# SobeyMIL/MVOC

Measured on AMD Instinct MI355X. Metric: UNet3D denoising steps/sec, 16x512^2 frames, inversion+compose, higher is better.
Workload: dtype f16

## Files before the change

mvoc_amd/csrc/attention.hip:

```cpp
#include <stdlib.h>

#include "common.h"

namespace {

typedef __fp16 fp16x4_t __attribute__((__vector_size__(4 * sizeof(__fp16))));
template <int D> struct FlashPitch { static constexpr int K = 2 * D + 16, V = D == 64 ? 192 : 320; };

struct AttnArgs {
  const half_t *q, *k, *v;
  half_t* out;
  long q_bs, q_ts, k_bs, k_ts, v_bs, v_ts, o_bs, o_ts;
  int nbatch, heads, tq, tk, kv_bdiv, causal;
  float scale_log2;
  long v2_off, o2_off;
  int qblocks;
};

__device__ __forceinline__ int vt_slot_group(int key) {
  return ((((key >> 5) * 2 + ((key >> 4) & 1)) * 2) + ((key >> 2) & 1));
}
__device__ __forceinline__ int vt_slot_elem(int key) { return ((key >> 3) & 1) * 4 + (key & 3); }

constexpr float FLASH_THR = 8.0f;

typedef float f32x2 __attribute__((ext_vector_type(2)));
__device__ __forceinline__ float flash_xhalf_max(float x) {
  const unsigned u = __builtin_bit_cast(unsigned, x);
  const auto sw = __builtin_amdgcn_permlane32_swap(u, u, false, false);
  return fmaxf(__builtin_bit_cast(float, (unsigned)sw[0]), __builtin_bit_cast(float, (unsigned)sw[1]));
}

template <int D, int NV>
#ifndef FLASH_MINW
#define FLASH_MINW 4
#endif
__global__ __launch_bounds__(256, (D == 64 && NV == 1) ? FLASH_MINW : 1) void flash_kernel(const AttnArgs p) {
  constexpr int KPITCH = FlashPitch<D>::K, VPITCH = FlashPitch<D>::V;
  constexpr int ND = D / 16, NT = D / 32, CPK = D / 8, NCH = 64 * CPK / 256;
  __shared__ __attribute__((aligned(16))) char smem[64 * KPITCH + NV * 64 * VPITCH];
  char* Ks = smem;
  char* Vs = smem + 64 * KPITCH;
  const int tid = threadIdx.x, lane = tid & 63;
  const int wave = __builtin_amdgcn_readfirstlane(tid >> 6);
  const int r = lane & 31, h = lane >> 5;
  const unsigned logical = xcd_remap(blockIdx.x, gridDim.x);
  const unsigned qb_ = logical % (unsigned)p.qblocks, hb_ = logical / (unsigned)p.qblocks;
  const int head = (int)(hb_ % (unsigned)p.heads), b = (int)(hb_ / (unsigned)p.heads);
  const int q0 = (int)qb_ * 128 + wave * 32;

  const half_t* qp = p.q + (long)b * p.q_bs + head * D;
  const int qrow = min(q0 + r, p.tq - 1);
  half8_t qf[ND];
#pragma unroll
  for (int s = 0; s < ND; ++s) qf[s] = *reinterpret_cast<const half8_t*>(qp + (long)qrow * p.q_ts + 16 * s + 8 * h);

  const char* kb = reinterpret_cast<const char*>(p.k + (long)(b / p.kv_bdiv) * p.k_bs + head * D);
  const char* vb = reinterpret_cast<const char*>(p.v + (long)(b / p.kv_bdiv) * p.v_bs + head * D);
  const unsigned k_rb = (unsigned)p.k_ts * 2u, v_rb = (unsigned)p.v_ts * 2u;
  unsigned koff[NCH], voff[NCH];
#pragma unroll
  for (int i = 0; i < NCH; ++i) {
    const int c = tid + i * 256;
    koff[i] = (unsigned)(c / CPK) * k_rb + (unsigned)(c % CPK) * 16u;
    voff[i] = (unsigned)(c / CPK) * v_rb + (unsigned)(c % CPK) * 16u;
  }

  f32x16 ot[NV][NT];
#pragma unroll
  for (int v = 0; v < NV; ++v)
#pragma unroll
    for (int dt = 0; dt < NT; ++dt)
#pragma unroll
      for (int e = 0; e < 16; ++e) ot[v][dt][e] = 0.f;
  float mrun = -INFINITY, lrun = 0.f;

  const int ntiles = (p.tk + 63) / 64;
  half8_t kreg[NCH], vreg[NV][NCH];
  auto gload = [&](int kt) {
    const char* kt_ = kb + (size_t)kt * 64u * k_rb;
    const char* vt_ = vb + (size_t)kt * 64u * v_rb;
    const bool ragged = __builtin_amdgcn_readfirstlane(kt * 64 + 64 > p.tk);
#pragma unroll
    for (int i = 0; i < NCH; ++i) {
      unsigned ko = koff[i], vo = voff[i];
      if (ragged) {
        const int c = tid + i * 256;
        const unsigned row = (unsigned)min(c / CPK, p.tk - 1 - kt * 64);
        ko = row * k_rb + (unsigned)(c % CPK) * 16u;
        vo = row * v_rb + (unsigned)(c % CPK) * 16u;
      }
      kreg[i] = *reinterpret_cast<const half8_t*>(kt_ + ko);
#pragma unroll
      for (int v = 0; v < NV; ++v) vreg[v][i] = *reinterpret_cast<const half8_t*>(vt_ + (size_t)v * (size_t)p.v2_off * 2u + vo);
    }
  };
  gload(0);
  for (int kt = 0; kt < ntiles; ++kt) {
    __syncthreads();
#pragma unroll
    for (int i = 0; i < NCH; ++i) {
      const int c = tid + i * 256;
      const int key = c / CPK, dc = c % CPK;
      *reinterpret_cast<half8_t*>(Ks + key * KPITCH + dc * 16) = kreg[i];
#pragma unroll
      for (int v = 0; v < NV; ++v)
        *reinterpret_cast<half8_t*>(Vs + v * 64 * VPITCH + key * VPITCH + dc * 16) = vreg[v][i];
    }
    __syncthreads();
    if (kt + 1 < ntiles) gload(kt + 1);

    f32x16 st[2];
#pragma unroll
    for (int t = 0; t < 2; ++t) {
#pragma unroll
      for (int e = 0; e < 16; ++e) st[t][e] = 0.f;
#pragma unroll
      for (int s = 0; s < ND; ++s) {
        const half8_t kf = *reinterpret_cast<const half8_t*>(Ks + (32 * t + r) * KPITCH + (16 * s + 8 * h) * 2);
        st[t] = __builtin_amdgcn_mfma_f32_32x32x16_f16(kf, qf[s], st[t], 0, 0, 0);
      }
    }
    if (__builtin_amdgcn_readfirstlane((kt == ntiles - 1) && (p.tk & 63))) {
#pragma unroll
      for (int t = 0; t < 2; ++t)
#pragma unroll
        for (int e = 0; e < 16; ++e)
          if (kt * 64 + 32 * t + 8 * (e >> 2) + 4 * h + (e & 3) >= p.tk) st[t][e] = -INFINITY;
    }
    if (p.causal) {
#pragma unroll
      for (int t = 0; t < 2; ++t)
#pragma unroll
        for (int e = 0; e < 16; ++e)
          if (kt * 64 + 32 * t + 8 * (e >> 2) + 4 * h + (e & 3) > q0 + r) st[t][e] = -INFINITY;
    }
    float mx = st[0][0];
#pragma unroll
    for (int t = 0; t < 2; ++t)
#pragma unroll
      for (int e = 0; e < 16; ++e) mx = fmaxf(mx, st[t][e]);
    mx = flash_xhalf_max(mx);
    if (__any((mx - mrun) * p.scale_log2 > FLASH_THR)) {
      const float mnew = fmaxf(mrun, mx);
      const float alpha = __builtin_amdgcn_exp2f((mrun - mnew) * p.scale_log2);
      mrun = mnew;
      lrun *= alpha;
#pragma unroll
      for (int v = 0; v < NV; ++v)
#pragma unroll
        for (int dt = 0; dt < NT; ++dt)
#pragma unroll
          for (int e = 0; e < 16; ++e) ot[v][dt][e] *= alpha;
    }
    const f32x2 sc2 = {p.scale_log2, p.scale_log2}, mc2 = {-mrun * p.scale_log2, -mrun * p.scale_log2};
#pragma unroll
    for (int t = 0; t < 2; ++t)
#pragma unroll
      for (int e = 0; e < 16; e += 2) {
        const f32x2 a = __builtin_elementwise_fma(f32x2{st[t][e], st[t][e + 1]}, sc2, mc2);
        st[t][e] = __builtin_amdgcn_exp2f(a[0]);
        st[t][e + 1] = __builtin_amdgcn_exp2f(a[1]);
      }

#pragma unroll
    for (int t = 0; t < 2; ++t)
#pragma unroll
      for (int s = 0; s < 2; ++s) {
        half8_t pf;
#pragma unroll
        for (int j = 0; j < 8; ++j) pf[j] = (half_t)st[t][8 * s + j];
#pragma unroll
        for (int j = 0; j < 4; ++j) lrun = __builtin_amdgcn_fdot2(half2_t{pf[2 * j], pf[2 * j + 1]}, half2_t{(half_t)1.f, (half_t)1.f}, lrun, false);
        const int krow = 32 * t + 16 * s + 4 * h + ((lane & 15) >> 2);
#pragma unroll
        for (int v = 0; v < NV; ++v)
#pragma unroll
          for (int dt = 0; dt < NT; ++dt) {
            const char* va = Vs + v * 64 * VPITCH + krow * VPITCH + (32 * dt + 16 * ((lane >> 4) & 1) + 4 * (lane & 3)) * 2;
            const fp16x4_t lo = __builtin_amdgcn_ds_read_tr16_b64_v4f16((__attribute__((address_space(3))) fp16x4_t*)va);
            const fp16x4_t hi = __builtin_amdgcn_ds_read_tr16_b64_v4f16((__attribute__((address_space(3))) fp16x4_t*)(va + 8 * VPITCH));
            half8_t vf;
#pragma unroll
            for (int e = 0; e < 4; ++e) {
              vf[e] = (half_t)lo[e];
              vf[4 + e] = (half_t)hi[e];
            }
            ot[v][dt] = __builtin_amdgcn_mfma_f32_32x32x16_f16(vf, pf, ot[v][dt], 0, 0, 0);
          }
      }
  }
  const float ltot = lrun + __shfl_xor(lrun, 32);
  const float inv = 1.0f / ltot;
  int lane_e = tid;
  asm volatile("" : "+v"(lane_e));
  const int r_e = lane_e & 31, h_e = (lane_e >> 5) & 1;
  if (q0 + r_e < p.tq) {
#pragma unroll
    for (int v = 0; v < NV; ++v) {
      half_t* op = p.out + v * p.o2_off + (long)b * p.o_bs + (long)(q0 + r_e) * p.o_ts + head * D;
#pragma unroll
      for (int dt = 0; dt < NT; ++dt)
#pragma unroll
        for (int q = 0; q < 4; ++q) {
          half4_t o;
#pragma unroll
          for (int e = 0; e < 4; ++e) o[e] = (half_t)(ot[v][dt][q * 4 + e] * inv);
          *reinterpret_cast<half4_t*>(op + 32 * dt + 8 * q + 4 * h_e) = o;
        }
    }
  }
}

#define F3_BAR()                         \
  do {                                   \
    __builtin_amdgcn_sched_barrier(0);   \
    __builtin_amdgcn_s_barrier();        \
    __builtin_amdgcn_sched_barrier(0);   \
  } while (0)
#define F3_FENCE() __builtin_amdgcn_sched_barrier(0)
#define F3_GRP(V, T)                                   \
  do {                                                 \
    __builtin_amdgcn_sched_group_barrier(0x008, 1, 0); \
    __builtin_amdgcn_sched_group_barrier(0x002, V, 0); \
    __builtin_amdgcn_sched_group_barrier(0x400, T, 0); \
  } while (0)
#define F3_RD(R) __builtin_amdgcn_sched_group_barrier(0x100, R, 0)
#ifdef MVOC_F3_STAMPS
__device__ unsigned long long f3_dbg[8];
#define F3_STAMP(i)                                                                      \
  do {                                                                                   \
    unsigned long long t_;                                                               \
    asm volatile("s_memtime %0\n\ts_waitcnt lgkmcnt(0)" : "=s"(t_)::"memory");          \
    if (blockIdx.x == 0 && tid == 0) { f3_acc[i] += t_ - f3_last; }                      \
    f3_last = t_;                                                                        \
  } while (0)
#else
#define F3_STAMP(i)
#endif
typedef unsigned u32x4 __attribute__((ext_vector_type(4)));
__device__ __forceinline__ void f3_dma(const u32x4 rsrc, unsigned voff, unsigned lds) {
  unsigned keep;
  asm volatile("s_mov_b32 %0, m0\n\ts_mov_b32 m0, %2\n\ts_nop 0\n\tbuffer_load_dwordx4 %1, %3, 0 offen lds\n\ts_mov_b32 m0, %0"
               : "=&s"(keep) : "v"(voff), "s"(lds), "s"(rsrc) : "memory");
}
__device__ __forceinline__ u32x4 f3_rsrc(const void* base, unsigned bytes) {
  const unsigned long long a = (unsigned long long)base;
  u32x4 r;
  r[0] = __builtin_amdgcn_readfirstlane((unsigned)a);
  r[1] = __builtin_amdgcn_readfirstlane((unsigned)(a >> 32));
  r[2] = __builtin_amdgcn_readfirstlane(bytes);
  r[3] = 0x00020000u;
  return r;
}
template <int N>
__device__ __forceinline__ void f3_wait_vm() {
  asm volatile("s_waitcnt vmcnt(%0)" ::"n"(N) : "memory");
}
#ifndef F3_W1
#define F3_W1 3
#endif
template <int NV>
__global__ __launch_bounds__(256, NV == 1 ? F3_W1 : 2) void flash3_kernel(const AttnArgs p) {
  constexpr int D = 64, NS = (NV == 1 && F3_W1 == 2) ? 4 : 3, TILE = 8192 * (1 + NV), PCS = 2 + 2 * NV;
  __shared__ __attribute__((aligned(1024))) char smem[NS * TILE];
#ifdef MVOC_F3_STAMPS
  unsigned long long f3_acc[6] = {0, 0, 0, 0, 0, 0}, f3_last = 0, f3_t0, f3_r0;
#endif
  const int tid = threadIdx.x, lane = tid & 63;
  const int wave = __builtin_amdgcn_readfirstlane(tid >> 6);
  const int r = lane & 31, h = lane >> 5;
#ifdef MVOC_F3_STAMPS
  asm volatile("s_memtime %0\n\ts_memrealtime %1\n\ts_waitcnt lgkmcnt(0)" : "=s"(f3_t0), "=s"(f3_r0)::"memory");
  f3_last = f3_t0;
#endif
  const unsigned logical = xcd_remap(blockIdx.x, gridDim.x);
  const unsigned qb_ = logical % (unsigned)p.qblocks, hb_ = logical / (unsigned)p.qblocks;
  const int head = (int)(hb_ % (unsigned)p.heads), b = (int)(hb_ / (unsigned)p.heads);
  const int q0 = (int)qb_ * 128 + wave * 32;
  const int nt = (p.tk + 63) >> 6;

  const unsigned k_rb = (unsigned)p.k_ts * 2u, v_rb = (unsigned)p.v_ts * 2u;
  const half_t* kb = p.k + (long)(b / p.kv_bdiv) * p.k_bs + head * D;
  const half_t* vb = p.v + (long)(b / p.kv_bdiv) * p.v_bs + head * D;
  const u32x4 rs_k = f3_rsrc(kb, (unsigned)(p.tk - 1) * k_rb + 128u);
  const u32x4 rs_v0 = f3_rsrc(vb, (unsigned)(p.tk - 1) * v_rb + 128u);
  const u32x4 rs_v1 = f3_rsrc(vb + p.v2_off, (unsigned)(p.tk - 1) * v_rb + 128u);
  unsigned ksrc[2], vsrc[2];
#pragma unroll
  for (int j = 0; j < 2; ++j) {
    const int key_l = 16 * wave + 8 * j + (lane >> 3), pc = lane & 7;
    ksrc[j] = (unsigned)key_l * k_rb + (unsigned)((pc ^ ((key_l >> 1) & 7)) * 16);
    vsrc[j] = (unsigned)key_l * v_rb + (unsigned)((pc ^ (((key_l >> 1) & 1) << 2)) * 16);
  }
  const unsigned ktile = 64u * k_rb, vtile = 64u * v_rb;
  const unsigned lds0 = (unsigned)(size_t)(__attribute__((address_space(3))) char*)smem;
  auto issue = [&](int tile, int so) {
    const unsigned base = lds0 + (unsigned)so + (unsigned)wave * 2048u;
#pragma unroll
    for (int j = 0; j < 2; ++j) f3_dma(rs_k, ksrc[j] + (unsigned)tile * ktile, base + j * 1024);
#pragma unroll
    for (int v = 0; v < NV; ++v)
#pragma unroll
      for (int j = 0; j < 2; ++j) f3_dma(v ? rs_v1 : rs_v0, vsrc[j] + (unsigned)tile * vtile, base + 8192 * (1 + v) + j * 1024);
  };
  const half_t* qp = p.q + (long)b * p.q_bs + head * D;
  const int qrow = min(q0 + r, p.tq - 1);
  half8_t qf[4];
#pragma unroll
  for (int s = 0; s < 4; ++s) qf[s] = *reinterpret_cast<const half8_t*>(qp + (long)qrow * p.q_ts + 16 * s + 8 * h);
  asm volatile("s_nop 4" ::: "memory");
  F3_FENCE();
#pragma unroll
  for (int t = 0; t < NS - 1; ++t) issue(t, t * TILE);
  F3_FENCE();

  f32x16 ot[NV][2];
#pragma unroll
  for (int v = 0; v < NV; ++v)
#pragma unroll
    for (int dt = 0; dt < 2; ++dt)
#pragma unroll
      for (int e = 0; e < 16; ++e) ot[v][dt][e] = 0.f;
  float mrun = -INFINITY, lrun = 0.f;
  f32x16 sa[2], sb[2];
  f32x16 zero16;
#pragma unroll
  for (int e = 0; e < 16; ++e) zero16[e] = 0.f;

  int kfo[4];
#pragma unroll
  for (int s = 0; s < 4; ++s) kfo[s] = r * 128 + (((2 * s + h) ^ ((r >> 1) & 7)) * 16);
  const int vq = (lane & 15) >> 2;
  int vfo[2];
#pragma unroll
  for (int dt = 0; dt < 2; ++dt) vfo[dt] = 8192 + (4 * h + vq) * 128 + (((32 * ((lane >> 4) & 1) + 8 * (lane & 3))) | ((dt ^ ((vq >> 1) & 1)) << 6));

  f3_wait_vm<(NS - 2) * PCS>();
  F3_BAR();
#pragma unroll
  for (int t = 0; t < 2; ++t) {
    sa[t] = zero16;
#pragma unroll
    for (int s = 0; s < 4; ++s) {
      const half8_t kf = *reinterpret_cast<const half8_t*>(smem + kfo[s] + 4096 * t);
      sa[t] = __builtin_amdgcn_mfma_f32_32x32x16_f16(kf, qf[s], sa[t], 0, 0, 0);
    }
  }
  int o_v = 0, o_k = TILE, o_w = (NS - 1) * TILE;

  auto body = [&](f32x16(&cur)[2], f32x16(&nxt)[2], const int t) {
    F3_STAMP(4);
    f3_wait_vm<(NS - 3) * PCS>();
    F3_BAR();
    F3_STAMP(0);
    issue(t + NS - 1, o_w);
    F3_FENCE();
    F3_STAMP(1);
    const char* Kn = smem + o_k;
    const char* Vc = smem + o_v;
    if (__builtin_amdgcn_readfirstlane((t == nt - 1) && (p.tk & 63))) {
#pragma unroll
      for (int tt = 0; tt < 2; ++tt)
#pragma unroll
        for (int e = 0; e < 16; ++e)
          if (t * 64 + 32 * tt + 8 * (e >> 2) + 4 * h + (e & 3) >= p.tk) cur[tt][e] = -INFINITY;
    }
    F3_FENCE();
    half8_t kf[2][4];
#pragma unroll
    for (int s = 0; s < 2; ++s)
#pragma unroll
      for (int tt = 0; tt < 2; ++tt) kf[tt][s] = *reinterpret_cast<const half8_t*>(Kn + kfo[s] + 4096 * tt);
    half8_t pf[2];
    half8_t vf[3][NV][2];
    auto vread = [&](const int f) {
#pragma unroll
      for (int v = 0; v < NV; ++v)
#pragma unroll
        for (int dt = 0; dt < 2; ++dt) {
          const char* va = Vc + 8192 * v + vfo[dt] + (32 * (f >> 1) + 16 * (f & 1)) * 128;
          const fp16x4_t lo = __builtin_amdgcn_ds_read_tr16_b64_v4f16((__attribute__((address_space(3))) fp16x4_t*)va);
          const fp16x4_t hi = __builtin_amdgcn_ds_read_tr16_b64_v4f16((__attribute__((address_space(3))) fp16x4_t*)(va + 8 * 128));
#pragma unroll
          for (int e = 0; e < 4; ++e) {
            vf[f % 3][v][dt][e] = (half_t)lo[e];
            vf[f % 3][v][dt][4 + e] = (half_t)hi[e];
          }
        }
    };
    vread(0);
    F3_FENCE();
    auto smma = [&](const int i) {
      const int tt = i & 1, s_ = i >> 1;
      nxt[tt] = __builtin_amdgcn_mfma_f32_32x32x16_f16(kf[tt][s_], qf[s_], s_ == 0 ? zero16 : nxt[tt], 0, 0, 0);
    };
    auto pvmma = [&](const int f, const int dt) {
#pragma unroll
      for (int v = 0; v < NV; ++v) ot[v][dt] = __builtin_amdgcn_mfma_f32_32x32x16_f16(vf[f % 3][v][dt], pf[f & 1], ot[v][dt], 0, 0, 0);
    };
    float mx = fmaxf(cur[0][0], cur[0][1]);
#pragma unroll
    for (int tt = 0; tt < 2; ++tt)
#pragma unroll
      for (int e = tt ? 0 : 2; e < 16; e += 2) mx = __builtin_fmaxf(__builtin_fmaxf(mx, cur[tt][e]), cur[tt][e + 1]);
    smma(0); smma(1); smma(2);
    if constexpr (NV == 2) smma(3);
    mx = flash_xhalf_max(mx);
    if constexpr (NV == 1) { F3_GRP(6, 0); F3_GRP(6, 0); F3_GRP(6, 0); }
    else { F3_GRP(4, 0); F3_GRP(5, 0); F3_GRP(4, 0); F3_GRP(5, 0); }
    F3_STAMP(2);
    if (__any((mx - mrun) * p.scale_log2 > FLASH_THR)) {
      const float mnew = fmaxf(mrun, mx);
      const float alpha = __builtin_amdgcn_exp2f((mrun - mnew) * p.scale_log2);
      mrun = mnew;
      lrun *= alpha;
#pragma unroll
      for (int v = 0; v < NV; ++v)
#pragma unroll
        for (int dt = 0; dt < 2; ++dt)
#pragma unroll
          for (int e = 0; e < 16; ++e) ot[v][dt][e] *= alpha;
    }
    F3_FENCE();
    const f32x2 sc2 = {p.scale_log2, p.scale_log2}, mc2 = {-mrun * p.scale_log2, -mrun * p.scale_log2};
#pragma unroll
    for (int s = 2; s < 4; ++s)
#pragma unroll
      for (int tt = 0; tt < 2; ++tt) kf[tt][s] = *reinterpret_cast<const half8_t*>(Kn + kfo[s] + 4096 * tt);
#pragma unroll
    for (int f = 0; f < 4; ++f) {
      const int tt = f >> 1, s_ = f & 1;
      if (f < 3) vread(f + 1);
      half8_t& pn = pf[f & 1];
      float x[8];
#pragma unroll
      for (int j = 0; j < 8; j += 2) {
        const f32x2 a = __builtin_elementwise_fma(f32x2{cur[tt][8 * s_ + j], cur[tt][8 * s_ + j + 1]}, sc2, mc2);
        x[j] = __builtin_amdgcn_exp2f(a[0]);
        x[j + 1] = __builtin_amdgcn_exp2f(a[1]);
      }
#pragma unroll
      for (int j = 0; j < 8; ++j) pn[j] = (half_t)x[j];
#pragma unroll
      for (int j = 0; j < 4; ++j) lrun = __builtin_amdgcn_fdot2(half2_t{pn[2 * j], pn[2 * j + 1]}, half2_t{(half_t)1.f, (half_t)1.f}, lrun, false);
      if (f == 0) {
        smma(NV == 1 ? 3 : 4); smma(NV == 1 ? 4 : 5);
        if constexpr (NV == 2) { smma(6); smma(7); } else smma(5);
      } else {
        pvmma(f - 1, 0); pvmma(f - 1, 1);
        if constexpr (NV == 1) { if (f < 3) smma(5 + f); }
      }
    }
    pvmma(3, 0);
    pvmma(3, 1);
    if constexpr (NV == 1) {
      F3_RD(8); F3_GRP(5, 3); F3_GRP(5, 2); F3_GRP(5, 3);
      F3_RD(4); F3_GRP(5, 2); F3_GRP(5, 3); F3_GRP(5, 2);
      F3_RD(4); F3_GRP(5, 3); F3_GRP(5, 2); F3_GRP(5, 3);
      F3_GRP(5, 2); F3_GRP(5, 3); F3_GRP(5, 2); F3_GRP(5, 2);
    } else {
      F3_RD(12); F3_GRP(3, 2); F3_GRP(3, 2); F3_GRP(3, 2); F3_GRP(3, 2);
      F3_RD(8); F3_GRP(3, 2); F3_GRP(3, 2); F3_GRP(3, 2); F3_GRP(3, 2);
      F3_RD(8); F3_GRP(3, 2); F3_GRP(3, 2); F3_GRP(3, 2); F3_GRP(3, 2);
      F3_GRP(3, 2); F3_GRP(3, 2); F3_GRP(3, 2); F3_GRP(3, 2);
      F3_GRP(3, 0); F3_GRP(3, 0); F3_GRP(3, 0); F3_GRP(3, 0);
    }
    F3_FENCE();
    F3_STAMP(3);
    const int o_ = o_v; o_v = o_k;
    o_k = o_k + TILE == NS * TILE ? 0 : o_k + TILE;
    o_w = o_;
  };
#pragma unroll 1
  for (int t = 0;; t += 2) {
    body(sa, sb, t);
    if (t + 1 >= nt) break;
    body(sb, sa, t + 1);
    if (t + 2 >= nt) break;
  }
  f3_wait_vm<0>();
#ifdef MVOC_F3_STAMPS
  if (blockIdx.x == 0 && tid == 0) {
    unsigned long long t1_, r1_;
    asm volatile("s_memtime %0\n\ts_memrealtime %1\n\ts_waitcnt lgkmcnt(0)" : "=s"(t1_), "=s"(r1_)::"memory");
    for (int i = 0; i < 5; ++i) f3_dbg[i] = f3_acc[i];
    f3_dbg[5] = t1_ - f3_t0;
    f3_dbg[7] = r1_ - f3_r0;
    f3_dbg[6] = (unsigned long long)nt;
  }
#endif

  const float ltot = lrun + __shfl_xor(lrun, 32);
  const float inv = 1.0f / ltot;
  if (q0 + r < p.tq) {
#pragma unroll
    for (int v = 0; v < NV; ++v) {
      half_t* op = p.out + v * p.o2_off + (long)b * p.o_bs + (long)(q0 + r) * p.o_ts + head * D;
#pragma unroll
      for (int dt = 0; dt < 2; ++dt)
#pragma unroll
        for (int q = 0; q < 4; ++q) {
          half4_t o;
#pragma unroll
          for (int e = 0; e < 4; ++e) o[e] = (half_t)(ot[v][dt][q * 4 + e] * inv);
          *reinterpret_cast<half4_t*>(op + 32 * dt + 8 * q + 4 * h) = o;
        }
    }
  }
}
#undef F3_BAR
#undef F3_FENCE
#undef F3_GRP
#undef F3_RD
#undef F3_STAMP

struct TAttnArgs {
  const half_t *q, *k, *v;
  half_t* out;
  long q_bs, q_ps, q_ts, k_bs, k_ps, k_ts, v_bs, v_ps, v_ts, o_bs, o_ps, o_ts;
  int nsample, hw, heads, frames;
  int logf, logp, pgroups;
  long ntask;
  float scale_log2;
};

constexpr int TVPITCH = 64;

__global__ __launch_bounds__(256) void tattn_kernel(const TAttnArgs p) {
  __shared__ __attribute__((aligned(16))) char smem[4 * 64 * TVPITCH];
  const int tid = threadIdx.x, lane = tid & 63, wave = tid >> 6;
  const int r = lane & 31, h = lane >> 5;
  char* Vs = smem + wave * 64 * TVPITCH;
  const int F = p.frames, logf = p.logf, P = 1 << p.logp;
  const long task = (long)blockIdx.x * 4 + wave;
  const bool active = task < p.ntask;
  const long tk = active ? task : p.ntask - 1;
  const int head = (int)(tk % p.heads);
  const long bp = tk / p.heads;
  const long smp = bp / p.pgroups, px0 = (bp % p.pgroups) << p.logp;
  const half8_t zero8 = {0, 0, 0, 0, 0, 0, 0, 0};
  auto row_px = [&](int row) { return (long)(P > 1 ? row >> logf : 0); };
  auto row_fr = [&](int row) { return P > 1 ? row & (F - 1) : row; };
  auto row_ok = [&](int row) { return (P > 1 || row < F) && px0 + row_px(row) < p.hw; };

  const half_t* qb = p.q + smp * p.q_bs + px0 * p.q_ps + head * 64;
  const half_t* kb = p.k + smp * p.k_bs + px0 * p.k_ps + head * 64;
  const half_t* vb = p.v + smp * p.v_bs + px0 * p.v_ps + head * 64;

#pragma unroll
  for (int i = 0; i < 4; ++i) {
    const int c = lane + 64 * i;
    const int key = c >> 3, dc = c & 7;
    half8_t vr = zero8;
    if (row_ok(key)) vr = *reinterpret_cast<const half8_t*>(vb + row_px(key) * p.v_ps + (long)row_fr(key) * p.v_ts + dc * 8);
    const int g = (((key >> 4) & 1) * 2) + ((key >> 2) & 1), j = vt_slot_elem(key);
#pragma unroll
    for (int e = 0; e < 8; ++e) {
      const int d = dc * 8 + e;
      *reinterpret_cast<half_t*>(Vs + d * TVPITCH + ((g ^ ((d >> 3) & 3)) * 16) + j * 2) = vr[e];
    }
  }
  f32x16 st;
#pragma unroll
  for (int e = 0; e < 16; ++e) st[e] = 0.f;
  const bool rok = row_ok(r);
  const long koff = row_px(r) * p.k_ps + (long)row_fr(r) * p.k_ts, qoff = row_px(r) * p.q_ps + (long)row_fr(r) * p.q_ts;
#pragma unroll
  for (int s = 0; s < 4; ++s) {
    half8_t kf = zero8, qf = zero8;
    if (rok) {
      kf = *reinterpret_cast<const half8_t*>(kb + koff + 16 * s + 8 * h);
      qf = *reinterpret_cast<const half8_t*>(qb + qoff + 16 * s + 8 * h);
    }
    st = __builtin_amdgcn_mfma_f32_32x32x16_f16(kf, qf, st, 0, 0, 0);
  }
  float mx = -INFINITY;
#pragma unroll
  for (int e = 0; e < 16; ++e) {
    const int key = 8 * (e >> 2) + 4 * h + (e & 3);
    const bool ok = P > 1 ? (key >> logf) == (r >> logf) : key < F;
    const float sv = ok ? st[e] * p.scale_log2 : -INFINITY;
    st[e] = sv;
    mx = fmaxf(mx, sv);
  }
  mx = fmaxf(mx, __shfl_xor(mx, 32));
  float ps = 0.f;
#pragma unroll
  for (int e = 0; e < 16; ++e) {
    const float pv = __builtin_amdgcn_exp2f(st[e] - mx);
    st[e] = pv;
    ps += pv;
  }
  ps += __shfl_xor(ps, 32);
  const float inv = 1.0f / ps;

  __syncthreads();
  f32x16 ot[2];
#pragma unroll
  for (int dt = 0; dt < 2; ++dt)
#pragma unroll
    for (int e = 0; e < 16; ++e) ot[dt][e] = 0.f;
#pragma unroll
  for (int s = 0; s < 2; ++s) {
    half8_t pf;
#pragma unroll
    for (int j = 0; j < 8; ++j) pf[j] = (half_t)st[8 * s + j];
    const int g = s * 2 + h;
#pragma unroll
    for (int dt = 0; dt < 2; ++dt) {
      const int d = 32 * dt + r;
      const half8_t vf = *reinterpret_cast<const half8_t*>(Vs + d * TVPITCH + ((g ^ ((d >> 3) & 3)) * 16));
      ot[dt] = __builtin_amdgcn_mfma_f32_32x32x16_f16(vf, pf, ot[dt], 0, 0, 0);
    }
  }
  if (active && rok) {
    half_t* op = p.out + smp * p.o_bs + (px0 + row_px(r)) * p.o_ps + (long)row_fr(r) * p.o_ts + head * 64;
#pragma unroll
    for (int dt = 0; dt < 2; ++dt)
#pragma unroll
      for (int q = 0; q < 4; ++q) {
        half4_t o;
#pragma unroll
        for (int e = 0; e < 4; ++e) o[e] = (half_t)(ot[dt][q * 4 + e] * inv);
        *reinterpret_cast<half4_t*>(op + 32 * dt + 8 * q + 4 * h) = o;
      }
  }
}

}

static const int g_f3_env = getenv("MVOC_FLASH3") ? atoi(getenv("MVOC_FLASH3")) : -1;

extern "C" int mvoc_flash_attn_f16(const mvoc_attn_desc* d, void* stream) {
  MVOC_REQUIRE(d && d->q && d->k && d->v && d->out, -1, "flash_attn: null operand");
  MVOC_REQUIRE(d->nbatch > 0 && d->heads > 0 && d->tq > 0 && d->tk > 0, -1, "flash_attn: empty problem");
  MVOC_REQUIRE(d->nbatch <= 65535 && d->heads <= 65535, -2, "flash_attn: grid too large");
  MVOC_REQUIRE(d->q_ts % 8 == 0 && d->k_ts % 8 == 0 && d->v_ts % 8 == 0 && d->o_ts % 4 == 0, -2,
               "flash_attn: row strides must keep 16-byte alignment");
  AttnArgs a;
  a.q = (const half_t*)d->q; a.k = (const half_t*)d->k; a.v = (const half_t*)d->v; a.out = (half_t*)d->out;
  a.q_bs = d->q_bs; a.q_ts = d->q_ts; a.k_bs = d->k_bs; a.k_ts = d->k_ts; a.v_bs = d->v_bs; a.v_ts = d->v_ts;
  a.o_bs = d->o_bs; a.o_ts = d->o_ts;
  a.nbatch = d->nbatch; a.heads = d->heads; a.tq = d->tq; a.tk = d->tk; a.kv_bdiv = d->kv_bdiv > 0 ? d->kv_bdiv : 1;
  const int hd = d->head_dim > 0 ? d->head_dim : 64;
  MVOC_REQUIRE(hd == 64 || hd == 96, -2, "flash_attn: head_dim (%d) must be 64 or 96", hd);
  MVOC_REQUIRE(!d->causal || d->tq == d->tk, -2, "flash_attn: the causal form is self-attention (tq == tk)");
  a.causal = d->causal;
  a.scale_log2 = (d->scale > 0.f ? d->scale : (hd == 64 ? 0.125f : 1.0f / sqrtf((float)hd))) * 1.4426950408889634f;
  hipStream_t s = (hipStream_t)stream;
  MvocProfScope prof(MVOC_FAM_FLASH, s, (d->v2 ? 2.0 : 1.0) * 4.0 * d->nbatch * d->heads * (double)d->tq * d->tk * hd);
  a.qblocks = (d->tq + 127) / 128;
  const long nblk = (long)a.qblocks * d->heads * d->nbatch;
  MVOC_REQUIRE(nblk < 0x7fffffffL, -2, "flash_attn: grid too large");
  dim3 grid((unsigned)nblk);
  a.v2_off = a.o2_off = 0;
  MVOC_REQUIRE(d->pipelined >= 0 && d->pipelined <= 2, -1, "flash_attn: pipelined must be 0 (by key count), 1 (never) or 2 (wherever it applies)");
  const int f3_mode = d->pipelined ? d->pipelined - 1 : g_f3_env;
  const bool pipelined = hd == 64 && !d->causal && (f3_mode >= 0 ? f3_mode != 0 : d->tk >= 2048);
  if (d->v2) {
    MVOC_REQUIRE(d->out2 && hd == 64, -2, "flash_attn: the paired form needs out2 and head_dim 64");
    a.v2_off = (const half_t*)d->v2 - a.v;
    a.o2_off = (half_t*)d->out2 - a.out;
    MVOC_REQUIRE(a.v2_off % 8 == 0 && a.o2_off % 4 == 0, -2, "flash_attn: v2 / out2 must keep 16-byte alignment");
    if (pipelined) hipLaunchKernelGGL((flash3_kernel<2>), grid, dim3(256), 0, s, a);
    else hipLaunchKernelGGL((flash_kernel<64, 2>), grid, dim3(256), 0, s, a);
  } else if (hd == 64) {
    if (pipelined) hipLaunchKernelGGL((flash3_kernel<1>), grid, dim3(256), 0, s, a);
    else hipLaunchKernelGGL((flash_kernel<64, 1>), grid, dim3(256), 0, s, a);
  } else {
    hipLaunchKernelGGL((flash_kernel<96, 1>), grid, dim3(256), 0, s, a);
  }
  return mvoc_check_launch("flash_kernel");
}

#ifdef MVOC_F3_STAMPS
extern "C" int mvoc_f3_stamps_read(unsigned long long* host8) {
  return hipMemcpyFromSymbol(host8, HIP_SYMBOL(f3_dbg), sizeof(unsigned long long) * 8) == hipSuccess ? 0 : -1;
}
#endif

extern "C" int mvoc_temporal_attn_f16(const mvoc_tattn_desc* d, void* stream) {
  MVOC_REQUIRE(d && d->q && d->k && d->v && d->out, -1, "temporal_attn: null operand");
  MVOC_REQUIRE(d->nsample > 0 && d->hw > 0 && d->heads > 0, -1, "temporal_attn: empty problem");
  MVOC_REQUIRE(d->frames >= 1 && d->frames <= 32, -2, "temporal_attn: frames (%d) must be in [1, 32]", d->frames);
  MVOC_REQUIRE(d->q_ts % 8 == 0 && d->k_ts % 8 == 0 && d->v_ts % 8 == 0 && d->o_ts % 4 == 0 && d->q_ps % 8 == 0 &&
                   d->k_ps % 8 == 0 && d->v_ps % 8 == 0 && d->o_ps % 4 == 0,
               -2, "temporal_attn: strides must keep 16-byte alignment");
  TAttnArgs a;
  a.q = (const half_t*)d->q; a.k = (const half_t*)d->k; a.v = (const half_t*)d->v; a.out = (half_t*)d->out;
  a.q_bs = d->q_bs; a.q_ps = d->q_ps; a.q_ts = d->q_ts; a.k_bs = d->k_bs; a.k_ps = d->k_ps; a.k_ts = d->k_ts;
  a.v_bs = d->v_bs; a.v_ps = d->v_ps; a.v_ts = d->v_ts; a.o_bs = d->o_bs; a.o_ps = d->o_ps; a.o_ts = d->o_ts;
  a.nsample = d->nsample; a.hw = d->hw; a.heads = d->heads; a.frames = d->frames;
  a.logf = d->frames == 8 ? 3 : d->frames == 16 ? 4 : 5;
  a.logp = d->frames == 8 ? 2 : d->frames == 16 ? 1 : 0;
  a.pgroups = (d->hw + (1 << a.logp) - 1) >> a.logp;
  a.ntask = (long)d->nsample * a.pgroups * d->heads;
  a.scale_log2 = 0.125f * 1.4426950408889634f;
  const long nblk = (a.ntask + 3) / 4;
  MVOC_REQUIRE(nblk < 0x7fffffffL, -2, "temporal_attn: grid too large");
  hipStream_t s = (hipStream_t)stream;
  MvocProfScope prof(MVOC_FAM_TATTN, s, 4.0 * (double)d->nsample * d->hw * d->heads * d->frames * 64 * 2);
  hipLaunchKernelGGL(tattn_kernel, dim3((unsigned)nblk), dim3(256), 0, s, a);
  return mvoc_check_launch("tattn_kernel");
}
```

Measured before the change: 21.99.

## Add KV-resident flash kernel for short keys and single-wave temporal attention kernel

Adds flashkv_kernel for cross-attention with at most 192 keys. Each 512-thread block loads the whole K/V of one head into LDS once, then loops over many query blocks with double-buffered Q loads and coalesced permlane-packed stores, instead of reloading K/V for every query block. Also adds tattn2_kernel for temporal attention with 8 or 16 frames, one wave per task with a swizzled V layout in LDS, and moves the per-tile flash body into a shared header. Both new paths are on by default through env flags, at the cost of extra code paths and the heuristic gating used to pick them.

```diff
diff --git a/mvoc_amd/csrc/attention.hip b/mvoc_amd/csrc/attention.hip
--- a/mvoc_amd/csrc/attention.hip
+++ b/mvoc_amd/csrc/attention.hip
@@ -15,6 +15,7 @@
   float scale_log2;
   long v2_off, o2_off;
   int qblocks;
+  int kv_tiles, kv_per, kv_nsplit, o16;
 };
 
 __device__ __forceinline__ int vt_slot_group(int key) {
@@ -25,6 +26,8 @@
 constexpr float FLASH_THR = 8.0f;
 
 typedef float f32x2 __attribute__((ext_vector_type(2)));
+typedef unsigned u32x2 __attribute__((ext_vector_type(2)));
+typedef unsigned u32x4 __attribute__((ext_vector_type(4)));
 __device__ __forceinline__ float flash_xhalf_max(float x) {
   const unsigned u = __builtin_bit_cast(unsigned, x);
   const auto sw = __builtin_amdgcn_permlane32_swap(u, u, false, false);
@@ -110,85 +113,7 @@
     __syncthreads();
     if (kt + 1 < ntiles) gload(kt + 1);
 
-    f32x16 st[2];
-#pragma unroll
-    for (int t = 0; t < 2; ++t) {
-#pragma unroll
-      for (int e = 0; e < 16; ++e) st[t][e] = 0.f;
-#pragma unroll
-      for (int s = 0; s < ND; ++s) {
-        const half8_t kf = *reinterpret_cast<const half8_t*>(Ks + (32 * t + r) * KPITCH + (16 * s + 8 * h) * 2);
-        st[t] = __builtin_amdgcn_mfma_f32_32x32x16_f16(kf, qf[s], st[t], 0, 0, 0);
-      }
-    }
-    if (__builtin_amdgcn_readfirstlane((kt == ntiles - 1) && (p.tk & 63))) {
-#pragma unroll
-      for (int t = 0; t < 2; ++t)
-#pragma unroll
-        for (int e = 0; e < 16; ++e)
-          if (kt * 64 + 32 * t + 8 * (e >> 2) + 4 * h + (e & 3) >= p.tk) st[t][e] = -INFINITY;
-    }
-    if (p.causal) {
-#pragma unroll
-      for (int t = 0; t < 2; ++t)
-#pragma unroll
-        for (int e = 0; e < 16; ++e)
-          if (kt * 64 + 32 * t + 8 * (e >> 2) + 4 * h + (e & 3) > q0 + r) st[t][e] = -INFINITY;
-    }
-    float mx = st[0][0];
-#pragma unroll
-    for (int t = 0; t < 2; ++t)
-#pragma unroll
-      for (int e = 0; e < 16; ++e) mx = fmaxf(mx, st[t][e]);
-    mx = flash_xhalf_max(mx);
-    if (__any((mx - mrun) * p.scale_log2 > FLASH_THR)) {
-      const float mnew = fmaxf(mrun, mx);
-      const float alpha = __builtin_amdgcn_exp2f((mrun - mnew) * p.scale_log2);
-      mrun = mnew;
-      lrun *= alpha;
-#pragma unroll
-      for (int v = 0; v < NV; ++v)
-#pragma unroll
-        for (int dt = 0; dt < NT; ++dt)
-#pragma unroll
-          for (int e = 0; e < 16; ++e) ot[v][dt][e] *= alpha;
-    }
-    const f32x2 sc2 = {p.scale_log2, p.scale_log2}, mc2 = {-mrun * p.scale_log2, -mrun * p.scale_log2};
-#pragma unroll
-    for (int t = 0; t < 2; ++t)
-#pragma unroll
-      for (int e = 0; e < 16; e += 2) {
-        const f32x2 a = __builtin_elementwise_fma(f32x2{st[t][e], st[t][e + 1]}, sc2, mc2);
-        st[t][e] = __builtin_amdgcn_exp2f(a[0]);
-        st[t][e + 1] = __builtin_amdgcn_exp2f(a[1]);
-      }
-
-#pragma unroll
-    for (int t = 0; t < 2; ++t)
-#pragma unroll
-      for (int s = 0; s < 2; ++s) {
-        half8_t pf;
-#pragma unroll
-        for (int j = 0; j < 8; ++j) pf[j] = (half_t)st[t][8 * s + j];
-#pragma unroll
-        for (int j = 0; j < 4; ++j) lrun = __builtin_amdgcn_fdot2(half2_t{pf[2 * j], pf[2 * j + 1]}, half2_t{(half_t)1.f, (half_t)1.f}, lrun, false);
-        const int krow = 32 * t + 16 * s + 4 * h + ((lane & 15) >> 2);
-#pragma unroll
-        for (int v = 0; v < NV; ++v)
-#pragma unroll
-          for (int dt = 0; dt < NT; ++dt) {
-            const char* va = Vs + v * 64 * VPITCH + krow * VPITCH + (32 * dt + 16 * ((lane >> 4) & 1) + 4 * (lane & 3)) * 2;
-            const fp16x4_t lo = __builtin_amdgcn_ds_read_tr16_b64_v4f16((__attribute__((address_space(3))) fp16x4_t*)va);
-            const fp16x4_t hi = __builtin_amdgcn_ds_read_tr16_b64_v4f16((__attribute__((address_space(3))) fp16x4_t*)(va + 8 * VPITCH));
-            half8_t vf;
-#pragma unroll
-            for (int e = 0; e < 4; ++e) {
-              vf[e] = (half_t)lo[e];
-              vf[4 + e] = (half_t)hi[e];
-            }
-            ot[v][dt] = __builtin_amdgcn_mfma_f32_32x32x16_f16(vf, pf, ot[v][dt], 0, 0, 0);
-          }
-      }
+#include "flash_tile.h"
   }
   const float ltot = lrun + __shfl_xor(lrun, 32);
   const float inv = 1.0f / ltot;
@@ -209,6 +134,120 @@
           *reinterpret_cast<half4_t*>(op + 32 * dt + 8 * q + 4 * h_e) = o;
         }
     }
+  }
+}
+
+__global__ __launch_bounds__(512, 4) void flashkv_kernel(const AttnArgs p) {
+  constexpr int D = 64, NV = 1, ND = 4, NT = 2, KPITCH = FlashPitch<D>::K, VPITCH = FlashPitch<D>::V, MAXK = 192;
+  __shared__ __attribute__((aligned(16))) char smem[MAXK * KPITCH + MAXK * VPITCH];
+  char* Ks_all = smem;
+  char* Vs_all = smem + MAXK * KPITCH;
+  const int tid = threadIdx.x, lane = tid & 63;
+  const int wave = __builtin_amdgcn_readfirstlane(tid >> 6);
+  const int r = lane & 31, h = lane >> 5;
+  const unsigned logical = xcd_remap(blockIdx.x, gridDim.x);
+  const unsigned split = logical % (unsigned)p.kv_nsplit, eh = logical / (unsigned)p.kv_nsplit;
+  const int head = (int)(eh % (unsigned)p.heads), entry = (int)(eh / (unsigned)p.heads);
+  const int ntiles = (p.tk + 63) / 64;
+
+  {
+    const char* kb = reinterpret_cast<const char*>(p.k + (long)entry * p.k_bs + head * D);
+    const char* vb = reinterpret_cast<const char*>(p.v + (long)entry * p.v_bs + head * D);
+    const unsigned k_rb = (unsigned)p.k_ts * 2u, v_rb = (unsigned)p.v_ts * 2u;
+    const int nchunk = ntiles * 64 * 8;
+    half8_t kreg[MAXK * 8 / 512], vreg[MAXK * 8 / 512];
+#pragma unroll
+    for (int i = 0; i < MAXK * 8 / 512; ++i) {
+      const int c = tid + i * 512;
+      if (c < nchunk) {
+        const unsigned row = (unsigned)min(c >> 3, p.tk - 1);
+        kreg[i] = *reinterpret_cast<const half8_t*>(kb + row * k_rb + (unsigned)(c & 7) * 16u);
+        vreg[i] = *reinterpret_cast<const half8_t*>(vb + row * v_rb + (unsigned)(c & 7) * 16u);
+      }
+    }
+#pragma unroll
+    for (int i = 0; i < MAXK * 8 / 512; ++i) {
+      const int c = tid + i * 512;
+      if (c < nchunk) {
+        *reinterpret_cast<half8_t*>(Ks_all + (c >> 3) * KPITCH + (c & 7) * 16) = kreg[i];
+        *reinterpret_cast<half8_t*>(Vs_all + (c >> 3) * VPITCH + (c & 7) * 16) = vreg[i];
+      }
+    }
+  }
+
+  const int tend = min(((int)split + 1) * p.kv_per, p.kv_tiles);
+  int t = (int)split * p.kv_per + (wave >> 2);
+  int b = entry * p.kv_bdiv + t / p.qblocks, qb = t % p.qblocks;
+  auto q_load = [&](half8_t(&dst)[4], int b_, int qb_) {
+    const int qrow = min(qb_ * 128 + (wave & 3) * 32 + r, p.tq - 1);
+    const half_t* qp = p.q + (long)b_ * p.q_bs + (long)qrow * p.q_ts + head * D + 8 * h;
+#pragma unroll
+    for (int s = 0; s < 4; ++s) dst[s] = *reinterpret_cast<const half8_t*>(qp + 16 * s);
+  };
+  half8_t qf[4], qn[4];
+  bool live = t < tend && b < p.nbatch;
+  if (live) q_load(qf, b, qb);
+  __syncthreads();
+
+  while (live) {
+    int tn = t + 2, bn = b, qbn = qb + 2;
+    while (qbn >= p.qblocks) { qbn -= p.qblocks; ++bn; }
+    const bool live_n = tn < tend && bn < p.nbatch;
+    if (live_n) q_load(qn, bn, qbn);
+
+    f32x16 ot[NV][NT];
+    const int q0 = qb * 128 + (wave & 3) * 32;
+#pragma unroll
+    for (int dt = 0; dt < 2; ++dt)
+#pragma unroll
+      for (int e = 0; e < 16; ++e) ot[0][dt][e] = 0.f;
+    float mrun = -INFINITY, lrun = 0.f;
+#pragma unroll 1
+    for (int kt = 0; kt < ntiles; ++kt) {
+      const char* Ks = Ks_all + kt * 64 * KPITCH;
+      const char* Vs = Vs_all + kt * 64 * VPITCH;
+#include "flash_tile.h"
+    }
+
+    const float ltot = lrun + __shfl_xor(lrun, 32);
+    const float inv = 1.0f / ltot;
+    const int qi = qb * 128 + (wave & 3) * 32 + r;
+    half_t* op = p.out + (long)b * p.o_bs + (long)qi * p.o_ts + head * D;
+    if (p.o16) {
+      u32x4 o[4];
+#pragma unroll
+      for (int dt = 0; dt < 2; ++dt)
+#pragma unroll
+        for (int j = 0; j < 2; ++j) {
+          half4_t ev, od;
+#pragma unroll
+          for (int e = 0; e < 4; ++e) {
+            ev[e] = (half_t)(ot[0][dt][(2 * j) * 4 + e] * inv);
+            od[e] = (half_t)(ot[0][dt][(2 * j + 1) * 4 + e] * inv);
+          }
+          const u32x2 eu = __builtin_bit_cast(u32x2, ev), ou = __builtin_bit_cast(u32x2, od);
+          const auto s0 = __builtin_amdgcn_permlane32_swap(eu[0], ou[0], false, false);
+          const auto s1 = __builtin_amdgcn_permlane32_swap(eu[1], ou[1], false, false);
+          o[2 * dt + j] = u32x4{(unsigned)s0[0], (unsigned)s1[0], (unsigned)s0[1], (unsigned)s1[1]};
+        }
+      if (qi < p.tq) {
+#pragma unroll
+        for (int c = 0; c < 4; ++c) *reinterpret_cast<u32x4*>(op + 16 * c + 8 * h) = o[c];
+      }
+    } else if (qi < p.tq) {
+#pragma unroll
+      for (int dt = 0; dt < 2; ++dt)
+#pragma unroll
+        for (int q = 0; q < 4; ++q) {
+          half4_t o;
+#pragma unroll
+          for (int e = 0; e < 4; ++e) o[e] = (half_t)(ot[0][dt][q * 4 + e] * inv);
+          *reinterpret_cast<half4_t*>(op + 32 * dt + 8 * q + 4 * h) = o;
+        }
+    }
+#pragma unroll
+    for (int s = 0; s < 4; ++s) qf[s] = qn[s];
+    t = tn; b = bn; qb = qbn; live = live_n;
   }
 }
 
@@ -238,7 +277,6 @@
 #else
 #define F3_STAMP(i)
 #endif
-typedef unsigned u32x4 __attribute__((ext_vector_type(4)));
 __device__ __forceinline__ void f3_dma(const u32x4 rsrc, unsigned voff, unsigned lds) {
   unsigned keep;
   asm volatile("s_mov_b32 %0, m0\n\ts_mov_b32 m0, %2\n\ts_nop 0\n\tbuffer_load_dwordx4 %1, %3, 0 offen lds\n\ts_mov_b32 m0, %0"
@@ -628,9 +666,139 @@
   }
 }
 
+__global__ __launch_bounds__(256, 6) void tattn2_kernel(const TAttnArgs p) {
+  __shared__ __attribute__((aligned(16))) char smem[4 * 32 * 128];
+  const int tid = threadIdx.x, lane = tid & 63, wave = tid >> 6;
+  const int r = lane & 31, h = lane >> 5;
+  char* Vs = smem + wave * 32 * 128;
+  const int F = p.frames, logf = p.logf;
+  const half8_t zero8 = {0, 0, 0, 0, 0, 0, 0, 0};
+  const long rpx = r >> logf;
+  const int rfr = r & (F - 1);
+  const int vkey = lane >> 3, vdc = lane & 7;
+
+  half8_t vr[4], kf[4], qf[4];
+  long px0, smp;
+  int head;
+  bool active;
+  {
+    const long task = (long)blockIdx.x * 4 + wave;
+    active = task < p.ntask;
+    const long tk = active ? task : p.ntask - 1;
+    head = (int)(tk % p.heads);
+    const long bp = tk / p.heads;
+    smp = bp / p.pgroups;
+    px0 = (bp % p.pgroups) << p.logp;
+    const half_t* qb = p.q + smp * p.q_bs + px0 * p.q_ps + head * 64;
+    const half_t* kb = p.k + smp * p.k_bs + px0 * p.k_ps + head * 64;
+    const half_t* vb = p.v + smp * p.v_bs + px0 * p.v_ps + head * 64;
+#pragma unroll
+    for (int i = 0; i < 4; ++i) {
+      const int key = vkey + 8 * i;
+      vr[i] = zero8;
+      if (px0 + (key >> logf) < p.hw) vr[i] = *reinterpret_cast<const half8_t*>(vb + (long)(key >> logf) * p.v_ps + (long)(key & (F - 1)) * p.v_ts + vdc * 8);
+    }
+    const bool rok = px0 + rpx < p.hw;
+    const long koff = rpx * p.k_ps + (long)rfr * p.k_ts, qoff = rpx * p.q_ps + (long)rfr * p.q_ts;
+#pragma unroll
+    for (int s = 0; s < 4; ++s) {
+      kf[s] = zero8;
+      qf[s] = zero8;
+      if (rok) {
+        kf[s] = *reinterpret_cast<const half8_t*>(kb + koff + 16 * s + 8 * h);
+        qf[s] = *reinterpret_cast<const half8_t*>(qb + qoff + 16 * s + 8 * h);
+      }
+    }
+  }
+
+  {
+#pragma unroll
+    for (int i = 0; i < 4; ++i) {
+      const int key = vkey + 8 * i;
+      *reinterpret_cast<half8_t*>(Vs + key * 128 + ((vdc ^ (((key >> 1) & 1) << 2)) * 16)) = vr[i];
+    }
+    f32x16 st;
+#pragma unroll
+    for (int e = 0; e < 16; ++e) st[e] = 0.f;
+#pragma unroll
+    for (int s = 0; s < 4; ++s) st = __builtin_amdgcn_mfma_f32_32x32x16_f16(kf[s], qf[s], st, 0, 0, 0);
+    float mx = -INFINITY;
+#pragma unroll
+    for (int e = 0; e < 16; ++e) {
+      const int key = 8 * (e >> 2) + 4 * h + (e & 3);
+      const bool ok = (key >> logf) == (r >> logf);
+      const float sv = ok ? st[e] * p.scale_log2 : -INFINITY;
+      st[e] = sv;
+      mx = fmaxf(mx, sv);
+    }
+    mx = fmaxf(mx, __shfl_xor(mx, 32));
+    float ps = 0.f;
+#pragma unroll
+    for (int e = 0; e < 16; ++e) {
+      const float pv = __builtin_amdgcn_exp2f(st[e] - mx);
+      st[e] = pv;
+      ps += pv;
+    }
+    ps += __shfl_xor(ps, 32);
+    const float inv = 1.0f / ps;
+
+    __builtin_amdgcn_fence(__ATOMIC_ACQ_REL, "wavefront");
+    __builtin_amdgcn_wave_barrier();
+    f32x16 ot[2];
+#pragma unroll
+    for (int dt = 0; dt < 2; ++dt)
+#pragma unroll
+      for (int e = 0; e < 16; ++e) ot[dt][e] = 0.f;
+    const int vq = (lane & 15) >> 2;
+#pragma unroll
+    for (int s = 0; s < 2; ++s) {
+      half8_t pf;
+#pragma unroll
+      for (int j = 0; j < 8; ++j) pf[j] = (half_t)st[8 * s + j];
+#pragma unroll
+      for (int dt = 0; dt < 2; ++dt) {
+        const char* va = Vs + (16 * s + 4 * h + vq) * 128 + ((32 * ((lane >> 4) & 1) + 8 * (lane & 3)) | ((dt ^ ((vq >> 1) & 1)) << 6));
+        const fp16x4_t lo = __builtin_amdgcn_ds_read_tr16_b64_v4f16((__attribute__((address_space(3))) fp16x4_t*)va);
+        const fp16x4_t hi = __builtin_amdgcn_ds_read_tr16_b64_v4f16((__attribute__((address_space(3))) fp16x4_t*)(va + 8 * 128));
+        half8_t vf;
+#pragma unroll
+        for (int e = 0; e < 4; ++e) {
+          vf[e] = (half_t)lo[e];
+          vf[4 + e] = (half_t)hi[e];
+        }
+        ot[dt] = __builtin_amdgcn_mfma_f32_32x32x16_f16(vf, pf, ot[dt], 0, 0, 0);
+      }
+    }
+    const bool rok = px0 + rpx < p.hw;
+    half_t* op = p.out + smp * p.o_bs + (px0 + rpx) * p.o_ps + (long)rfr * p.o_ts + head * 64;
+    u32x4 o[4];
+#pragma unroll
+    for (int dt = 0; dt < 2; ++dt)
+#pragma unroll
+      for (int j = 0; j < 2; ++j) {
+        half4_t ev, od;
+#pragma unroll
+        for (int e = 0; e < 4; ++e) {
+          ev[e] = (half_t)(ot[dt][(2 * j) * 4 + e] * inv);
+          od[e] = (half_t)(ot[dt][(2 * j + 1) * 4 + e] * inv);
+        }
+        const u32x2 eu = __builtin_bit_cast(u32x2, ev), ou = __builtin_bit_cast(u32x2, od);
+        const auto s0 = __builtin_amdgcn_permlane32_swap(eu[0], ou[0], false, false);
+        const auto s1 = __builtin_amdgcn_permlane32_swap(eu[1], ou[1], false, false);
+        o[2 * dt + j] = u32x4{(unsigned)s0[0], (unsigned)s1[0], (unsigned)s0[1], (unsigned)s1[1]};
+      }
+    if (active && rok) {
+#pragma unroll
+      for (int c = 0; c < 4; ++c) *reinterpret_cast<u32x4*>(op + 16 * c + 8 * h) = o[c];
+    }
+  }
+}
+
 }
 
 static const int g_f3_env = getenv("MVOC_FLASH3") ? atoi(getenv("MVOC_FLASH3")) : -1;
+static const int g_kv_env = getenv("MVOC_FLASH_KV") ? atoi(getenv("MVOC_FLASH_KV")) : 1;
+static const int g_t2_env = getenv("MVOC_TATTN2") ? atoi(getenv("MVOC_TATTN2")) : 1;
 
 extern "C" int mvoc_flash_attn_f16(const mvoc_attn_desc* d, void* stream) {
   MVOC_REQUIRE(d && d->q && d->k && d->v && d->out, -1, "flash_attn: null operand");
@@ -655,9 +823,26 @@
   MVOC_REQUIRE(nblk < 0x7fffffffL, -2, "flash_attn: grid too large");
   dim3 grid((unsigned)nblk);
   a.v2_off = a.o2_off = 0;
+  a.kv_tiles = a.kv_per = a.kv_nsplit = a.o16 = 0;
   MVOC_REQUIRE(d->pipelined >= 0 && d->pipelined <= 2, -1, "flash_attn: pipelined must be 0 (by key count), 1 (never) or 2 (wherever it applies)");
   const int f3_mode = d->pipelined ? d->pipelined - 1 : g_f3_env;
   const bool pipelined = hd == 64 && !d->causal && (f3_mode >= 0 ? f3_mode != 0 : d->tk >= 2048);
+  const long kv_tiles = (long)(a.kv_bdiv < d->nbatch ? a.kv_bdiv : d->nbatch) * a.qblocks;
+  const long entries = (d->nbatch + a.kv_bdiv - 1) / a.kv_bdiv, eh = entries * d->heads;
+  const bool kv_wins = a.qblocks >= 32 && kv_tiles >= 256 && eh * kv_tiles >= 8192;
+  if (d->pipelined == 0 && g_f3_env < 0 && g_kv_env != 0 && hd == 64 && !d->v2 && !d->causal && d->tk <= 192 && kv_tiles >= 8 &&
+      (kv_wins || g_kv_env == 2)) {
+    long nsplit = 1024 / eh < kv_tiles / 4 ? 1024 / eh : kv_tiles / 4;
+    if (nsplit < 1) nsplit = 1;
+    if (eh * nsplit < 256) nsplit = (256 + eh - 1) / eh < kv_tiles ? (256 + eh - 1) / eh : kv_tiles;
+    a.kv_tiles = (int)kv_tiles;
+    a.kv_per = (int)((kv_tiles + nsplit - 1) / nsplit);
+    a.kv_nsplit = (int)((kv_tiles + a.kv_per - 1) / a.kv_per);
+    a.o16 = d->o_ts % 8 == 0 && d->o_bs % 8 == 0 && (size_t)d->out % 16 == 0;
+    MVOC_REQUIRE(eh * a.kv_nsplit < 0x7fffffffL, -2, "flash_attn: grid too large");
+    hipLaunchKernelGGL(flashkv_kernel, dim3((unsigned)(eh * a.kv_nsplit)), dim3(512), 0, s, a);
+    return mvoc_check_launch("flashkv_kernel");
+  }
   if (d->v2) {
     MVOC_REQUIRE(d->out2 && hd == 64, -2, "flash_attn: the paired form needs out2 and head_dim 64");
     a.v2_off = (const half_t*)d->v2 - a.v;
@@ -701,6 +886,10 @@
   MVOC_REQUIRE(nblk < 0x7fffffffL, -2, "temporal_attn: grid too large");
   hipStream_t s = (hipStream_t)stream;
   MvocProfScope prof(MVOC_FAM_TATTN, s, 4.0 * (double)d->nsample * d->hw * d->heads * d->frames * 64 * 2);
+  if (g_t2_env != 0 && (d->frames == 8 || d->frames == 16) && d->o_ts % 8 == 0 && d->o_ps % 8 == 0 && d->o_bs % 8 == 0 && (size_t)d->out % 16 == 0) {
+    hipLaunchKernelGGL(tattn2_kernel, dim3((unsigned)nblk), dim3(256), 0, s, a);
+    return mvoc_check_launch("tattn2_kernel");
+  }
   hipLaunchKernelGGL(tattn_kernel, dim3((unsigned)nblk), dim3(256), 0, s, a);
   return mvoc_check_launch("tattn_kernel");
 }
diff --git a/mvoc_amd/csrc/flash_tile.h b/mvoc_amd/csrc/flash_tile.h
--- /dev/null
+++ b/mvoc_amd/csrc/flash_tile.h
@@ -0,0 +1,79 @@
+    f32x16 st[2];
+#pragma unroll
+    for (int t = 0; t < 2; ++t) {
+#pragma unroll
+      for (int e = 0; e < 16; ++e) st[t][e] = 0.f;
+#pragma unroll
+      for (int s = 0; s < ND; ++s) {
+        const half8_t kf = *reinterpret_cast<const half8_t*>(Ks + (32 * t + r) * KPITCH + (16 * s + 8 * h) * 2);
+        st[t] = __builtin_amdgcn_mfma_f32_32x32x16_f16(kf, qf[s], st[t], 0, 0, 0);
+      }
+    }
+    if (__builtin_amdgcn_readfirstlane((kt == ntiles - 1) && (p.tk & 63))) {
+#pragma unroll
+      for (int t = 0; t < 2; ++t)
+#pragma unroll
+        for (int e = 0; e < 16; ++e)
+          if (kt * 64 + 32 * t + 8 * (e >> 2) + 4 * h + (e & 3) >= p.tk) st[t][e] = -INFINITY;
+    }
+    if (p.causal) {
+#pragma unroll
+      for (int t = 0; t < 2; ++t)
+#pragma unroll
+        for (int e = 0; e < 16; ++e)
+          if (kt * 64 + 32 * t + 8 * (e >> 2) + 4 * h + (e & 3) > q0 + r) st[t][e] = -INFINITY;
+    }
+    float mx = st[0][0];
+#pragma unroll
+    for (int t = 0; t < 2; ++t)
+#pragma unroll
+      for (int e = 0; e < 16; ++e) mx = fmaxf(mx, st[t][e]);
+    mx = flash_xhalf_max(mx);
+    if (__any((mx - mrun) * p.scale_log2 > FLASH_THR)) {
+      const float mnew = fmaxf(mrun, mx);
+      const float alpha = __builtin_amdgcn_exp2f((mrun - mnew) * p.scale_log2);
+      mrun = mnew;
+      lrun *= alpha;
+#pragma unroll
+      for (int v = 0; v < NV; ++v)
+#pragma unroll
+        for (int dt = 0; dt < NT; ++dt)
+#pragma unroll
+          for (int e = 0; e < 16; ++e) ot[v][dt][e] *= alpha;
+    }
+    const f32x2 sc2 = {p.scale_log2, p.scale_log2}, mc2 = {-mrun * p.scale_log2, -mrun * p.scale_log2};
+#pragma unroll
+    for (int t = 0; t < 2; ++t)
+#pragma unroll
+      for (int e = 0; e < 16; e += 2) {
+        const f32x2 a = __builtin_elementwise_fma(f32x2{st[t][e], st[t][e + 1]}, sc2, mc2);
+        st[t][e] = __builtin_amdgcn_exp2f(a[0]);
+        st[t][e + 1] = __builtin_amdgcn_exp2f(a[1]);
+      }
+
+#pragma unroll
+    for (int t = 0; t < 2; ++t)
+#pragma unroll
+      for (int s = 0; s < 2; ++s) {
+        half8_t pf;
+#pragma unroll
+        for (int j = 0; j < 8; ++j) pf[j] = (half_t)st[t][8 * s + j];
+#pragma unroll
+        for (int j = 0; j < 4; ++j) lrun = __builtin_amdgcn_fdot2(half2_t{pf[2 * j], pf[2 * j + 1]}, half2_t{(half_t)1.f, (half_t)1.f}, lrun, false);
+        const int krow = 32 * t + 16 * s + 4 * h + ((lane & 15) >> 2);
+#pragma unroll
+        for (int v = 0; v < NV; ++v)
+#pragma unroll
+          for (int dt = 0; dt < NT; ++dt) {
+            const char* va = Vs + v * 64 * VPITCH + krow * VPITCH + (32 * dt + 16 * ((lane >> 4) & 1) + 4 * (lane & 3)) * 2;
+            const fp16x4_t lo = __builtin_amdgcn_ds_read_tr16_b64_v4f16((__attribute__((address_space(3))) fp16x4_t*)va);
+            const fp16x4_t hi = __builtin_amdgcn_ds_read_tr16_b64_v4f16((__attribute__((address_space(3))) fp16x4_t*)(va + 8 * VPITCH));
+            half8_t vf;
+#pragma unroll
+            for (int e = 0; e < 4; ++e) {
+              vf[e] = (half_t)lo[e];
+              vf[4 + e] = (half_t)hi[e];
+            }
+            ot[v][dt] = __builtin_amdgcn_mfma_f32_32x32x16_f16(vf, pf, ot[v][dt], 0, 0, 0);
+          }
+      }
```

New measurement: 22.10, median of 6. About the same (+0.5%).
